# FocoosAI/focoos

Hardware: NVIDIA H100
Metric: images/sec fai-detr-l bs=32 640x640 inference (higher is better)
Workload: dtype f32 (storage and accumulation; every conv/linear product = 3 f16 wgmma products, error ~2^-21)

## Files before the change

focoos_b200/csrc/conv_tc.cu:

```cuda
#include <cuda.h>

#include <cstdlib>
#include <type_traits>

#include "common.cuh"
#include "tma.cuh"
#include "wgmma.cuh"

namespace fb200 {

namespace tc {

constexpr int BLOCK_M = 128;
constexpr int STAGING_BYTES = BLOCK_M * 128;
constexpr int NUM_THREADS = 384;
constexpr int CONSUMER_WARPS = 8;

struct PairOut { __half hi, lo; };
template <typename T> struct is_pair { static constexpr bool value = false; };
template <> struct is_pair<PairOut> { static constexpr bool value = true; };

struct KParams {
  const float* scale; const float* bias; const void* res;
  int act, Cout;
  int KH, KW, pad, cchunks;
  int w_batched;
  int lo_off;
  int w_seg;
  int BW, BH, tiles_w, tiles_h;
  int Ho, Wo;
  int x_pitch;
  int stride2;
  int num_k_blocks;
  int n_tiles, total_tiles;
  float* rowmax;
};

__device__ __forceinline__ void consumer_bar() { asm volatile("bar.sync 1, 256;" ::: "memory"); }

template <int BLOCK_K>
__device__ __forceinline__ uint64_t make_smem_desc(uint32_t smem_addr) {
  uint64_t d = 0;
  d |= (uint64_t)((smem_addr & 0x3FFFFu) >> 4);
  d |= (uint64_t)1 << 16;
  d |= (uint64_t)((8 * BLOCK_K * 2) >> 4) << 32;
  d |= (uint64_t)(BLOCK_K == 64 ? 1 : 2) << 62;
  return d;
}

template <bool GELU>
__device__ __forceinline__ float act1(float v, int act) {
  if constexpr (GELU) return 0.5f * v * (1.f + erff(v * 0.70710678118654752440f));
  switch (act & 15) {
    case FB200_ACT_RELU: return fmaxf(v, 0.f);
    case FB200_ACT_SILU: return __fdividef(v, 1.f + __expf(-v));
    default: return v;
  }
}

__device__ __forceinline__ void atomic_max_float(float* addr, float v) {
  if (v >= 0.f) atomicMax(reinterpret_cast<int*>(addr), __float_as_int(v));
  else atomicMin(reinterpret_cast<unsigned int*>(addr), __float_as_uint(v));
}

struct AccThread {
  int ct;
  int g;
  int r0;
  int cq;
};
__device__ __forceinline__ AccThread acc_thread() {
  const int ct = threadIdx.x - 128, lane = threadIdx.x & 31;
  return {ct, ct >> 7, (ct >> 7) * 64 + ((ct & 127) >> 5) * 16 + (lane >> 2), 2 * (lane & 3)};
}

template <typename TOut>
__device__ __forceinline__ int staging_offset(int row, int lc) {
  if constexpr (is_pair<TOut>::value) return row * 64 + ((((lc >> 3) ^ ((row >> 1) & 3)) << 4) | ((lc & 7) * 2));
  else if constexpr (sizeof(TOut) == 2) return row * 128 + ((((lc >> 3) ^ (row & 7)) << 4) | ((lc & 7) * 2));
  else return row * 128 + ((((lc >> 2) ^ (row & 7)) << 4) | ((lc & 3) * 4));
}

template <typename TOut>
__device__ __forceinline__ void staging_store(uint8_t* stg, int off, float v0, float v1) {
  if constexpr (is_pair<TOut>::value) {
    const __half2 hi = __floats2half2_rn(v0, v1);
    const float2 hf = __half22float2(hi);
    *reinterpret_cast<__half2*>(stg + off) = hi;
    *reinterpret_cast<__half2*>(stg + STAGING_BYTES / 2 + off) = __floats2half2_rn(v0 - hf.x, v1 - hf.y);
  } else if constexpr (sizeof(TOut) == 2) {
    *reinterpret_cast<__half2*>(stg + off) = __floats2half2_rn(v0, v1);
  } else {
    *reinterpret_cast<float2*>(stg + off) = make_float2(v0, v1);
  }
}

template <int NSTG, typename F>
__device__ __forceinline__ void staging_open(int ct, F&& then) {
  if (ct == 0) {
    tma_store_wait_read<NSTG - 1>();
    then();
  }
  consumer_bar();
}
template <typename TOut>
__device__ __forceinline__ void staging_close(int ct, const uint8_t* stg, const CUtensorMap* tmap_d, const CUtensorMap* tmap_d2, int n, int w0, int h0, int img) {
  fence_proxy_async();
  consumer_bar();
  if (ct == 0) {
    tma_store_4d(tmap_d, stg, n, w0, h0, img);
    if constexpr (is_pair<TOut>::value) tma_store_4d(tmap_d2, stg + STAGING_BYTES / 2, n, w0, h0, img);
    tma_store_commit();
  }
}

template <int BLOCK_K, bool FS> __host__ __device__ constexpr int a_stage_bytes() { return (FS ? 2 : 1) * BLOCK_M * BLOCK_K * 2; }
template <int BLOCK_N, int BLOCK_K, bool FS> __host__ __device__ constexpr int b_stage_bytes() { return (FS ? 2 : 1) * BLOCK_N * BLOCK_K * 2; }
template <int BLOCK_N, int STAGES, int BLOCK_K, int NSTG, bool FS> constexpr int smem_bytes() {
  return STAGES * (a_stage_bytes<BLOCK_K, FS>() + b_stage_bytes<BLOCK_N, BLOCK_K, FS>()) + NSTG * STAGING_BYTES + (2 * STAGES + 1) * 8 + 1024 ;
}

template <int BLOCK_N, int STAGES, typename TOut, int BLOCK_K, int NSTG, bool GELU, bool FS>
__global__ void __launch_bounds__(NUM_THREADS, 1)
conv_tc_kernel(const __grid_constant__ CUtensorMap tmap_a, const __grid_constant__ CUtensorMap tmap_b,
               const __grid_constant__ CUtensorMap tmap_d, const __grid_constant__ CUtensorMap tmap_r,
               const __grid_constant__ CUtensorMap tmap_d2, const __grid_constant__ CUtensorMap tmap_r2, const KParams p) {
  constexpr bool PAIR = is_pair<TOut>::value;
  static_assert(BLOCK_K == 32 || BLOCK_K == 64, "one swizzle row per channel chunk");
  extern __shared__ __align__(1024) uint8_t smem_raw[];
  uint8_t* smem = reinterpret_cast<uint8_t*>((reinterpret_cast<uintptr_t>(smem_raw) + 1023) & ~uintptr_t(1023));
  constexpr int A_STAGE_BYTES = a_stage_bytes<BLOCK_K, FS>();
  constexpr int B_STAGE_BYTES = b_stage_bytes<BLOCK_N, BLOCK_K, FS>();
  constexpr int A_HALF = BLOCK_M * BLOCK_K * 2;
  constexpr int B_HALF = BLOCK_N * BLOCK_K * 2;
  uint8_t* smem_a = smem;
  uint8_t* smem_b = smem + STAGES * A_STAGE_BYTES;
  uint8_t* staging = smem_b + STAGES * B_STAGE_BYTES;
  uint64_t* full_bar = reinterpret_cast<uint64_t*>(staging + NSTG * STAGING_BYTES);
  uint64_t* empty_bar = full_bar + STAGES;
  uint64_t* res_bar = empty_bar + STAGES;

  constexpr int CHUNK_COLS = 128 / (int)sizeof(TOut);
  constexpr int NCHUNKS = (BLOCK_N + CHUNK_COLS - 1) / CHUNK_COLS;
  constexpr int RES_SLOTS_A = A_STAGE_BYTES / STAGING_BYTES;
  constexpr int RES_SLOTS = RES_SLOTS_A + B_STAGE_BYTES / STAGING_BYTES;
  constexpr bool RES_RING = RES_SLOTS > 0;
  const bool res_ring = RES_RING && p.res != nullptr && p.rowmax == nullptr;
  auto res_slot = [&](int s, int slot) -> uint8_t* {
    return slot < RES_SLOTS_A ? smem_a + s * A_STAGE_BYTES + slot * STAGING_BYTES : smem_b + s * B_STAGE_BYTES + (slot - RES_SLOTS_A) * STAGING_BYTES;
  };
  auto chunks_of = [&](int n0) { return min(NCHUNKS, (p.Cout - n0 + CHUNK_COLS - 1) / CHUNK_COLS); };

  const int warp = threadIdx.x >> 5, lane = threadIdx.x & 31;
  if (threadIdx.x == 0) {
    asm volatile("prefetch.tensormap [%0];" ::"l"(&tmap_a) : "memory");
    asm volatile("prefetch.tensormap [%0];" ::"l"(&tmap_b) : "memory");
    asm volatile("prefetch.tensormap [%0];" ::"l"(&tmap_d) : "memory");
    for (int i = 0; i < STAGES; ++i) { mbar_init(&full_bar[i], 1); mbar_init(&empty_bar[i], CONSUMER_WARPS); }
    if constexpr (!RES_RING) mbar_init(res_bar, 1);
    fence_barrier_init();
  }
  __syncthreads();
  const int tiles_per_img = p.tiles_w * p.tiles_h;
  struct TileXY { int n0, img, h0, w0; };
  auto tile_of = [&](int t) {
    TileXY r;
    r.n0 = (t % p.n_tiles) * BLOCK_N;
    const int mt = t / p.n_tiles;
    r.img = mt / tiles_per_img;
    const int rem = mt - r.img * tiles_per_img;
    r.h0 = (rem / p.tiles_w) * p.BH;
    r.w0 = (rem % p.tiles_w) * p.BW;
    return r;
  };

  if (warp < 4) {
    if (threadIdx.x != 0) return;
    const uint32_t a_bytes = (uint32_t)(p.BW * p.BH * BLOCK_K * 2);
    auto load_a = [&](uint64_t* bar, void* dst, int c, int kh, int kw, int h0, int w0, int img) {
      if (!p.stride2) {
        tma_load_4d(&tmap_a, bar, dst, c, w0 + kw - p.pad, h0 + kh - p.pad, img);
      } else if (p.stride2 == 2) {
        tma_load_4d(&tmap_a, bar, dst, c, 2 * w0 + kw - p.pad, 2 * h0 + kh - p.pad, img);
      } else {
        const int th = kh - p.pad, tw = kw - p.pad;
        tma_load_5d(&tmap_a, bar, dst, (tw & 1) * p.x_pitch + c, w0 + (tw >> 1), th & 1, h0 + (th >> 1), img);
      }
    };
    auto load_b = [&](uint64_t* bar, void* dst, int k, int n0, int img) {
      if (p.w_batched) tma_load_3d(&tmap_b, bar, dst, k, n0, img);
      else tma_load_2d(&tmap_b, bar, dst, k, n0);
    };
    int stage = 0;
    uint32_t phase = 0;
    for (int t = blockIdx.x; t < p.total_tiles; t += gridDim.x) {
      const TileXY tc = tile_of(t);
      for (int kb = 0; kb < p.num_k_blocks; ++kb) {
        mbar_wait(&empty_bar[stage], phase ^ 1);
        const int tap = kb / p.cchunks, cc = kb - tap * p.cchunks;
        const int kh = tap / p.KW, kw = tap - kh * p.KW;
        uint8_t* dst_a = smem_a + stage * A_STAGE_BYTES;
        uint8_t* dst_b = smem_b + stage * B_STAGE_BYTES;
        if constexpr (FS) {
          const int k_hi = tap * 3 * p.w_seg + cc * BLOCK_K, k_lo = k_hi + p.w_seg;
          mbar_arrive_expect_tx(&full_bar[stage], 2u * a_bytes + (uint32_t)B_STAGE_BYTES);
          load_a(&full_bar[stage], dst_a, cc * BLOCK_K, kh, kw, tc.h0, tc.w0, tc.img);
          load_a(&full_bar[stage], dst_a + A_HALF, p.lo_off + cc * BLOCK_K, kh, kw, tc.h0, tc.w0, tc.img);
          load_b(&full_bar[stage], dst_b, k_hi, tc.n0, tc.img);
          load_b(&full_bar[stage], dst_b + B_HALF, k_lo, tc.n0, tc.img);
        } else {
          mbar_arrive_expect_tx(&full_bar[stage], a_bytes + (uint32_t)B_STAGE_BYTES);
          load_a(&full_bar[stage], dst_a, cc * BLOCK_K, kh, kw, tc.h0, tc.w0, tc.img);
          load_b(&full_bar[stage], dst_b, kb * BLOCK_K, tc.n0, tc.img);
        }
        if (++stage == STAGES) { stage = 0; phase ^= 1; }
      }
      if constexpr (RES_RING) if (res_ring) {
        const int nch = chunks_of(tc.n0);
        for (int ch = 0; ch < nch; ++ch) {
          const int slot = ch % RES_SLOTS;
          if (slot == 0) {
            mbar_wait(&empty_bar[stage], phase ^ 1);
            mbar_arrive_expect_tx(&full_bar[stage], (uint32_t)(min(RES_SLOTS, nch - ch) * p.BW * p.BH * 128));
          }
          uint8_t* dst = res_slot(stage, slot);
          tma_load_4d(&tmap_r, &full_bar[stage], dst, tc.n0 + ch * CHUNK_COLS, tc.w0, tc.h0, tc.img);
          if constexpr (PAIR) tma_load_4d(&tmap_r2, &full_bar[stage], dst + STAGING_BYTES / 2, tc.n0 + ch * CHUNK_COLS, tc.w0, tc.h0, tc.img);
          if (slot == RES_SLOTS - 1 || ch == nch - 1) {
            if (++stage == STAGES) { stage = 0; phase ^= 1; }
          }
        }
      }
    }
    return;
  }

  const AccThread th = acc_thread();
  constexpr int NACC = BLOCK_N / 2;
  const bool post = (p.act & FB200_ACT_RESIDUAL_AFTER) != 0;
  const bool has_res = p.res != nullptr;
  float acc[NACC];
  int stage = 0;
  uint32_t phase = 0, res_phase = 0, chunk_ctr = 0;
  for (int t = blockIdx.x; t < p.total_tiles; t += gridDim.x) {
    const TileXY tc = tile_of(t);
    int prev = -1;
    for (int kb = 0; kb < p.num_k_blocks; ++kb) {
      mbar_wait(&full_bar[stage], phase);
      const uint32_t sa = smem_u32(smem_a + stage * A_STAGE_BYTES) + (uint32_t)(th.g * 64 * BLOCK_K * 2);
      const uint32_t sb = smem_u32(smem_b + stage * B_STAGE_BYTES);
      const uint64_t da = make_smem_desc<BLOCK_K>(sa), db = make_smem_desc<BLOCK_K>(sb);
      wgmma_fence();
#pragma unroll
      for (int k = 0; k < BLOCK_K / 16; ++k) {
        const uint64_t ko = (uint64_t)(k * 2);
        Wgmma<BLOCK_N, 0>::mma(acc, da + ko, db + ko, (kb > 0 || k > 0) ? 1u : 0u);
        if constexpr (FS) {
          const uint64_t da_lo = make_smem_desc<BLOCK_K>(sa + A_HALF), db_lo = make_smem_desc<BLOCK_K>(sb + B_HALF);
          Wgmma<BLOCK_N, 0>::mma(acc, da + ko, db_lo + ko, 1u);
          Wgmma<BLOCK_N, 0>::mma(acc, da_lo + ko, db + ko, 1u);
        }
      }
      wgmma_commit();
      wgmma_wait<1>();
      if (prev >= 0 && lane == 0) mbar_arrive(&empty_bar[prev]);
      prev = stage;
      if (++stage == STAGES) { stage = 0; phase ^= 1; }
    }
    wgmma_wait<0>();
    if (prev >= 0 && lane == 0) mbar_arrive(&empty_bar[prev]);

    auto scale_of = [&](int n) { return (p.scale && n < p.Cout) ? __ldg(p.scale + n) : 1.f; };
    auto bias_of = [&](int n) { return (p.bias && n < p.Cout) ? __ldg(p.bias + n) : 0.f; };
    auto row_valid = [&](int row, int64_t& pix) {
      const int bh = row / p.BW, bw = row - bh * p.BW;
      const int ho = tc.h0 + bh, wo = tc.w0 + bw;
      pix = ((int64_t)tc.img * p.Ho + ho) * p.Wo + wo;
      return row < p.BW * p.BH && ho < p.Ho && wo < p.Wo;
    };
    if (p.rowmax) {
      float m[2] = {-INFINITY, -INFINITY};
#pragma unroll
      for (int j = 0; j < BLOCK_N / 8; ++j) {
#pragma unroll
        for (int e = 0; e < 2; ++e) {
          const int n = tc.n0 + 8 * j + th.cq + e;
          if (n < p.Cout) {
            const float s = scale_of(n), b = bias_of(n);
            m[0] = fmaxf(m[0], fmaf(acc[4 * j + e], s, b));
            m[1] = fmaxf(m[1], fmaf(acc[4 * j + 2 + e], s, b));
          }
        }
      }
#pragma unroll
      for (int h = 0; h < 2; ++h) {
        m[h] = fmaxf(m[h], __shfl_xor_sync(0xffffffffu, m[h], 1));
        m[h] = fmaxf(m[h], __shfl_xor_sync(0xffffffffu, m[h], 2));
        int64_t pix;
        if ((lane & 3) == 0 && row_valid(th.r0 + 8 * h, pix)) atomic_max_float(p.rowmax + pix, m[h]);
      }
      continue;
    }
    const int nch = chunks_of(tc.n0);
#pragma unroll
    for (int ch = 0; ch < NCHUNKS; ++ch) {
      const int c0 = ch * CHUNK_COLS;
      if (ch >= nch) break;
      uint8_t* stg = staging + (chunk_ctr % NSTG) * STAGING_BYTES;
      const uint8_t* res = stg;
      staging_open<NSTG>(th.ct, [&] {
        if constexpr (!RES_RING) if (has_res) {
          mbar_arrive_expect_tx(res_bar, (uint32_t)(p.BW * p.BH * 128));
          tma_load_4d(&tmap_r, res_bar, stg, tc.n0 + c0, tc.w0, tc.h0, tc.img);
          if constexpr (PAIR) tma_load_4d(&tmap_r2, res_bar, stg + STAGING_BYTES / 2, tc.n0 + c0, tc.w0, tc.h0, tc.img);
        }
      });
      if constexpr (RES_RING) {
        if (res_ring) {
          if (ch % RES_SLOTS == 0) mbar_wait(&full_bar[stage], phase);
          res = res_slot(stage, ch % RES_SLOTS);
        }
      } else if (has_res) {
        mbar_wait(res_bar, res_phase);
        res_phase ^= 1;
      }
#pragma unroll
      for (int jj = 0; jj < CHUNK_COLS / 8; ++jj) {
        const int j = c0 / 8 + jj;
        if (j >= BLOCK_N / 8) break;
        const int lc = 8 * jj + th.cq;
        const int n = tc.n0 + c0 + lc;
        const float s0 = scale_of(n), s1 = scale_of(n + 1), b0 = bias_of(n), b1 = bias_of(n + 1);
#pragma unroll
        for (int h = 0; h < 2; ++h) {
          const int row = th.r0 + 8 * h;
          float v0 = fmaf(acc[4 * j + 2 * h], s0, b0), v1 = fmaf(acc[4 * j + 2 * h + 1], s1, b1);
          const int off = staging_offset<TOut>(row, lc);
          auto add_residual = [&]() {
            if (!has_res) return;
            if constexpr (PAIR) {
              const float2 fh = __half22float2(*reinterpret_cast<const __half2*>(res + off));
              const float2 fl = __half22float2(*reinterpret_cast<const __half2*>(res + STAGING_BYTES / 2 + off));
              v0 += fh.x + fl.x;
              v1 += fh.y + fl.y;
            } else if constexpr (sizeof(TOut) == 2) {
              const float2 f = __half22float2(*reinterpret_cast<const __half2*>(res + off));
              v0 += f.x;
              v1 += f.y;
            } else {
              const float2 f = *reinterpret_cast<const float2*>(res + off);
              v0 += f.x;
              v1 += f.y;
            }
          };
          if (!post) add_residual();
          v0 = act1<GELU>(v0, p.act);
          v1 = act1<GELU>(v1, p.act);
          if (post) add_residual();
          staging_store<TOut>(stg, off, v0, v1);
        }
      }
      if constexpr (RES_RING) {
        if (res_ring && (ch % RES_SLOTS == RES_SLOTS - 1 || ch == nch - 1)) {
          __syncwarp();
          if (lane == 0) mbar_arrive(&empty_bar[stage]);
          if (++stage == STAGES) { stage = 0; phase ^= 1; }
        }
      }
      staging_close<TOut>(th.ct, stg, &tmap_d, &tmap_d2, tc.n0 + c0, tc.w0, tc.h0, tc.img);
      ++chunk_ctr;
    }
  }
  if (th.ct == 0) tma_store_wait_all();
}

constexpr int SC_BW = 16, SC_BH = 8;
constexpr int SC_BOX_ROWS = SC_BW * (SC_BH + 2);
constexpr int SC_BOX_BYTES = SC_BOX_ROWS * 64;
constexpr int SC_STAGE_BYTES = 2 * 3 * SC_BOX_BYTES;
constexpr int SC_STAGES = 2;
template <int BLOCK_N> __host__ __device__ constexpr int sc_w_bytes() { return 9 * 2 * BLOCK_N * 64; }
template <int BLOCK_N> constexpr int sc_smem_bytes() {
  return sc_w_bytes<BLOCK_N>() + SC_STAGES * SC_STAGE_BYTES + 2 * STAGING_BYTES + (2 * SC_STAGES + 1) * 8 + 1024 ;
}

template <int BLOCK_N, typename TOut>
__global__ void __launch_bounds__(NUM_THREADS, 1)
conv_tc_smallc_kernel(const __grid_constant__ CUtensorMap tmap_a, const __grid_constant__ CUtensorMap tmap_b,
                      const __grid_constant__ CUtensorMap tmap_d, const __grid_constant__ CUtensorMap tmap_d2, const KParams p) {
  constexpr int W_BYTES = sc_w_bytes<BLOCK_N>();
  constexpr int W_TAP = 2 * BLOCK_N * 64;
  extern __shared__ __align__(1024) uint8_t smem_raw[];
  uint8_t* smem = reinterpret_cast<uint8_t*>((reinterpret_cast<uintptr_t>(smem_raw) + 1023) & ~uintptr_t(1023));
  uint8_t* smem_w = smem;
  uint8_t* smem_a = smem_w + W_BYTES;
  uint8_t* staging = smem_a + SC_STAGES * SC_STAGE_BYTES;
  uint64_t* full_bar = reinterpret_cast<uint64_t*>(staging + 2 * STAGING_BYTES);
  uint64_t* empty_bar = full_bar + SC_STAGES;
  uint64_t* w_bar = empty_bar + SC_STAGES;
  constexpr int CHUNK_COLS = 32;
  constexpr int NCHUNKS = BLOCK_N / CHUNK_COLS;

  const int warp = threadIdx.x >> 5, lane = threadIdx.x & 31;
  if (threadIdx.x == 0) {
    asm volatile("prefetch.tensormap [%0];" ::"l"(&tmap_a) : "memory");
    asm volatile("prefetch.tensormap [%0];" ::"l"(&tmap_d) : "memory");
    for (int i = 0; i < SC_STAGES; ++i) { mbar_init(&full_bar[i], 1); mbar_init(&empty_bar[i], CONSUMER_WARPS); }
    mbar_init(w_bar, 1);
    fence_barrier_init();
  }
  __syncthreads();
  const int tiles_per_img = p.tiles_w * p.tiles_h;
  struct TileXY { int img, h0, w0; };
  auto tile_of = [&](int t) {
    TileXY r;
    r.img = t / tiles_per_img;
    const int rem = t - r.img * tiles_per_img;
    r.h0 = (rem / p.tiles_w) * SC_BH;
    r.w0 = (rem % p.tiles_w) * SC_BW;
    return r;
  };

  if (warp < 4) {
    if (threadIdx.x != 0) return;
    mbar_arrive_expect_tx(w_bar, (uint32_t)W_BYTES);
    for (int tap = 0; tap < 9; ++tap) {
      tma_load_2d(&tmap_b, w_bar, smem_w + tap * W_TAP, tap * 3 * p.w_seg, 0);
      tma_load_2d(&tmap_b, w_bar, smem_w + tap * W_TAP + W_TAP / 2, tap * 3 * p.w_seg + p.w_seg, 0);
    }
    int stage = 0;
    uint32_t phase = 0;
    for (int t = blockIdx.x; t < p.total_tiles; t += gridDim.x) {
      const TileXY tc = tile_of(t);
      mbar_wait(&empty_bar[stage], phase ^ 1);
      mbar_arrive_expect_tx(&full_bar[stage], (uint32_t)SC_STAGE_BYTES);
      uint8_t* dst = smem_a + stage * SC_STAGE_BYTES;
      for (int kw = 0; kw < 3; ++kw) {
        tma_load_4d(&tmap_a, &full_bar[stage], dst + kw * SC_BOX_BYTES, 0, tc.w0 + kw - 1, tc.h0 - 1, tc.img);
        tma_load_4d(&tmap_a, &full_bar[stage], dst + (3 + kw) * SC_BOX_BYTES, p.lo_off, tc.w0 + kw - 1, tc.h0 - 1, tc.img);
      }
      if (++stage == SC_STAGES) { stage = 0; phase ^= 1; }
    }
    return;
  }

  const AccThread th = acc_thread();
  float acc[BLOCK_N / 2];
  float sc[BLOCK_N / 4], bi[BLOCK_N / 4];
#pragma unroll
  for (int j = 0; j < BLOCK_N / 8; ++j)
#pragma unroll
    for (int e = 0; e < 2; ++e) {
      const int n = 8 * j + th.cq + e;
      sc[2 * j + e] = p.scale ? __ldg(p.scale + n) : 1.f;
      bi[2 * j + e] = p.bias ? __ldg(p.bias + n) : 0.f;
    }
  mbar_wait(w_bar, 0);
  const uint32_t sw = smem_u32(smem_w);
  int stage = 0;
  uint32_t phase = 0, chunk_ctr = 0;
  for (int t = blockIdx.x; t < p.total_tiles; t += gridDim.x) {
    const TileXY tc = tile_of(t);
    mbar_wait(&full_bar[stage], phase);
    const uint32_t sa = smem_u32(smem_a + stage * SC_STAGE_BYTES) + (uint32_t)(th.g * 64 * 64);
    wgmma_fence();
#pragma unroll
    for (int tap = 0; tap < 9; ++tap) {
      const int kh = tap / 3, kw = tap - 3 * (tap / 3);
      const uint32_t a_tap = sa + (uint32_t)(kw * SC_BOX_BYTES + kh * SC_BW * 64);
      const uint64_t da = make_smem_desc<32>(a_tap), da_lo = make_smem_desc<32>(a_tap + 3 * SC_BOX_BYTES);
      const uint64_t db = make_smem_desc<32>(sw + tap * W_TAP), db_lo = make_smem_desc<32>(sw + tap * W_TAP + W_TAP / 2);
#pragma unroll
      for (int k = 0; k < 2; ++k) {
        const uint64_t ko = (uint64_t)(k * 2);
        Wgmma<BLOCK_N, 0>::mma(acc, da + ko, db + ko, (tap > 0 || k > 0) ? 1u : 0u);
        Wgmma<BLOCK_N, 0>::mma(acc, da + ko, db_lo + ko, 1u);
        Wgmma<BLOCK_N, 0>::mma(acc, da_lo + ko, db + ko, 1u);
      }
    }
    wgmma_commit();
    wgmma_wait<0>();
    if (lane == 0) mbar_arrive(&empty_bar[stage]);
    if (++stage == SC_STAGES) { stage = 0; phase ^= 1; }

#pragma unroll
    for (int ch = 0; ch < NCHUNKS; ++ch) {
      uint8_t* stg = staging + (chunk_ctr & 1) * STAGING_BYTES;
      staging_open<2>(th.ct, [] {});
#pragma unroll
      for (int jj = 0; jj < CHUNK_COLS / 8; ++jj) {
        const int j = ch * (CHUNK_COLS / 8) + jj;
        const int lc = 8 * jj + th.cq;
#pragma unroll
        for (int h = 0; h < 2; ++h) {
          const int row = th.r0 + 8 * h;
          const float v0 = act1<false>(fmaf(acc[4 * j + 2 * h], sc[2 * j], bi[2 * j]), p.act);
          const float v1 = act1<false>(fmaf(acc[4 * j + 2 * h + 1], sc[2 * j + 1], bi[2 * j + 1]), p.act);
          staging_store<TOut>(stg, staging_offset<TOut>(row, lc), v0, v1);
        }
      }
      staging_close<TOut>(th.ct, stg, &tmap_d, &tmap_d2, ch * CHUNK_COLS, tc.w0, tc.h0, tc.img);
      ++chunk_ctr;
    }
  }
  if (th.ct == 0) tma_store_wait_all();
}

static void choose_tile(int Ho, int Wo, int* BW, int* BH) {
  double best = -1.0;
  for (int bw = 1; bw <= (Wo < 128 ? Wo : 128); ++bw) {
    int bh = 128 / bw;
    if (bh > Ho) bh = Ho;
    if (bh < 1) continue;
    const double tiles = (double)((Wo + bw - 1) / bw) * (double)((Ho + bh - 1) / bh);
    const double eff = (double)Wo * Ho / (tiles * 128.0);
    if (eff > best + 1e-9 || (eff > best - 1e-9 && bw > *BW)) { best = eff; *BW = bw; *BH = bh; }
  }
}

struct OutMaps { CUtensorMap d, d2, r, r2; };
static int encode_out_maps(OutMaps* m, const ConvParams& p, int Wo, int Ho, int B, int BW, int BH, uint64_t batch_stride) {
  const bool pair = p.out_dtype == FB200_F16PAIR, f32 = p.out_dtype == FB200_F32;
  const CUtensorMapDataType dt = f32 ? CU_TENSOR_MAP_DATA_TYPE_FLOAT32 : CU_TENSOR_MAP_DATA_TYPE_FLOAT16;
  const int elt = f32 ? 4 : 2;
  const CUtensorMapSwizzle swz = pair ? CU_TENSOR_MAP_SWIZZLE_64B : CU_TENSOR_MAP_SWIZZLE_128B;
  const uint64_t OP = (uint64_t)p.out_pitch, RP = (uint64_t)p.res_pitch;
  const uint64_t dims[4] = {(uint64_t)p.Cout, (uint64_t)Wo, (uint64_t)Ho, (uint64_t)B};
  const uint64_t str[4] = {1, OP, OP * Wo, batch_stride}, rstr[4] = {1, RP, RP * Wo, RP * Wo * Ho};
  const uint32_t box[4] = {(uint32_t)(pair || f32 ? 32 : 64), (uint32_t)BW, (uint32_t)BH, 1};
  int rc = encode(&m->d, dt, elt, 4, p.out, dims, str, box, pair ? "conv_tc: D(hi)" : "conv_tc: D", swz);
  if (rc) return rc;
  m->d2 = m->d;
  if (pair) rc = encode(&m->d2, dt, elt, 4, static_cast<__half*>(p.out) + p.out_lo_off, dims, str, box, "conv_tc: D(lo)", swz);
  if (rc) return rc;
  m->r = m->d; m->r2 = m->d2;
  if (!p.res) return FB200_OK;
  rc = encode(&m->r, dt, elt, 4, const_cast<void*>(p.res), dims, rstr, box, pair ? "conv_tc: R(hi)" : "conv_tc: R", swz);
  if (rc || !pair) return rc;
  return encode(&m->r2, dt, elt, 4, const_cast<__half*>(static_cast<const __half*>(p.res)) + p.res_lo_off, dims, rstr, box, "conv_tc: R(lo)", swz);
}

static bool smallc_fits(const ConvParams& p) {
  return p.split3 && p.Cin == 3 * 32 && (p.Cout == 32 || p.Cout == 64) && p.KH == 3 && p.KW == 3 && p.stride == 1 && p.pad == 1 &&
         !p.res && !p.rowmax && p.w_bs == 0 && (p.out_dtype == FB200_F32 || p.out_dtype == FB200_F16PAIR);
}

static int conv2d_tc_smallc(const ConvParams& p, cudaStream_t st) {
  KParams kp{};
  kp.scale = p.scale; kp.bias = p.bias; kp.act = p.act; kp.Cout = p.Cout;
  kp.lo_off = (int)p.x_lo_off;
  kp.w_seg = 32;
  kp.tiles_w = (p.Wo + SC_BW - 1) / SC_BW; kp.tiles_h = (p.Ho + SC_BH - 1) / SC_BH; kp.Ho = p.Ho; kp.Wo = p.Wo;
  const int64_t total = (int64_t)p.B * kp.tiles_w * kp.tiles_h;
  if (total > 0x7fffffffLL) { set_error("conv_tc: too many tiles (%lld)", (long long)total); return FB200_ERR_UNSUPPORTED; }
  kp.total_tiles = (int)total;
  CUtensorMap ta, tb;
  OutMaps om;
  const uint64_t P = (uint64_t)p.x_pitch;
  {
    const uint64_t dims[4] = {(uint64_t)kp.lo_off + 32, (uint64_t)p.W, (uint64_t)p.H, (uint64_t)p.B};
    const uint64_t str[4] = {1, P, P * p.W, P * p.W * p.H};
    const uint32_t box[4] = {32, SC_BW, SC_BH + 2, 1};
    int rc = encode(&ta, CU_TENSOR_MAP_DATA_TYPE_FLOAT16, 2, 4, const_cast<void*>(p.x), dims, str, box, "conv_tc: A(patch)", CU_TENSOR_MAP_SWIZZLE_64B);
    if (rc) return rc;
  }
  {
    const uint64_t dims[2] = {(uint64_t)p.K, (uint64_t)p.Cout};
    const uint64_t str[2] = {1, (uint64_t)p.K};
    const uint32_t box[2] = {32, (uint32_t)p.Cout};
    int rc = encode(&tb, CU_TENSOR_MAP_DATA_TYPE_FLOAT16, 2, 2, const_cast<void*>(p.w), dims, str, box, "conv_tc: W", CU_TENSOR_MAP_SWIZZLE_64B);
    if (rc) return rc;
  }
  if (int rc = encode_out_maps(&om, p, p.Wo, p.Ho, p.B, SC_BW, SC_BH, (uint64_t)p.out_bs)) return rc;
  auto run = [&](auto blockn_tag, auto out_tag) -> int {
    constexpr int BN_ = decltype(blockn_tag)::value;
    return launch_persistent<conv_tc_smallc_kernel<BN_, decltype(out_tag)>, sc_smem_bytes<BN_>()>("conv_tc_smallc_kernel", kp.total_tiles, NUM_THREADS, st, ta, tb,
                                                                                                 om.d, om.d2, kp);
  };
  typedef std::integral_constant<int, 32> N32;
  typedef std::integral_constant<int, 64> N64;
  const bool outp = p.out_dtype == FB200_F16PAIR;
  if (p.Cout == 32) return outp ? run(N32{}, PairOut{}) : run(N32{}, float{});
  return outp ? run(N64{}, PairOut{}) : run(N64{}, float{});
}

}

bool conv2d_tc_supported(const ConvParams& p, int x_dtype, int out_dtype) {
  if (x_dtype != FB200_F16) return false;
  if (out_dtype != FB200_F16 && out_dtype != FB200_F32 && out_dtype != FB200_F16PAIR) return false;
  if (p.split3 && out_dtype == FB200_F16) return false;
  const int Clog = p.split3 ? p.Cin / 3 : p.Cin;
  if (out_dtype == FB200_F16PAIR) {
    if (!p.split3 || p.rowmax || p.w_bs != 0 || p.Cout % 8 != 0) return false;
    if ((p.out_lo_off * 2) % 16 != 0 || (p.out_pitch * 2) % 16 != 0 || (p.out_bs * 2) % 16 != 0) return false;
    if (p.res && ((p.res_lo_off * 2) % 16 != 0 || (p.res_pitch * 2) % 16 != 0 || p.Cout % 32 != 0)) return false;
  }
  if (p.split3 && (p.x_lo_off * 2) % 16 != 0) return false;
  if (Clog % 32 != 0 || p.x_pitch % 8 != 0) return false;
  if (p.split3 && p.Cin % 3 != 0) return false;
  if ((reinterpret_cast<uintptr_t>(p.x) | reinterpret_cast<uintptr_t>(p.w) | reinterpret_cast<uintptr_t>(p.out)) & 15) return false;
  const int oelt = out_dtype == FB200_F32 ? 4 : 2;
  if ((p.out_pitch * oelt) % 16 != 0) return false;
  if (!p.rowmax && (p.Cout * oelt) % 16 != 0) return false;
  if (p.res && ((p.res_pitch * oelt) % 16 != 0 || (reinterpret_cast<uintptr_t>(p.res) & 15))) return false;
  if (p.res && out_dtype != FB200_F16PAIR && p.Cout % (128 / oelt) != 0) return false;
  if (p.KH != p.KW) return false;
  if (p.w_bs != 0 && (p.w_bs * 2) % 16 != 0) return false;
  if ((p.act & 15) == FB200_ACT_GELU && (out_dtype != FB200_F16 || Clog % 64 != 0)) return false;
  if ((p.act & 15) == FB200_ACT_SIGMOID) return false;
  if ((p.out_bs * oelt) % 16 != 0) return false;
  if (p.stride == 1) return (2 * p.pad == p.KH - 1) || (p.KH == 1 && p.pad == 0);
  if (p.stride == 2) {
    if (p.KH == 3 && p.pad == 1) return true;
    return p.KH == 2 && p.pad == 0 && p.H % 2 == 0 && p.W % 2 == 0;
  }
  return false;
}

int conv2d_tc(const ConvParams& p, cudaStream_t st) {
  using namespace tc;
  if (smallc_fits(p)) return conv2d_tc_smallc(p, st);
  KParams kp;
  kp.scale = p.scale; kp.bias = p.bias; kp.res = p.res; kp.act = p.act; kp.Cout = p.Cout;
  kp.KH = p.KH; kp.KW = p.KW; kp.pad = p.pad;
  const int Clog = p.split3 ? p.Cin / 3 : p.Cin;
  const int BK = (Clog % 64 == 0) ? 64 : 32;
  kp.lo_off = p.split3 ? (int)p.x_lo_off : Clog;
  kp.w_seg = Clog;
  const CUtensorMapSwizzle swz = BK == 64 ? CU_TENSOR_MAP_SWIZZLE_128B : CU_TENSOR_MAP_SWIZZLE_64B;
  kp.cchunks = Clog / BK; kp.x_pitch = p.x_pitch;
  kp.stride2 = (p.stride != 2) ? 0 : (p.H % 2 == 0 && p.W % 2 == 0) ? 1 : 2;
  kp.num_k_blocks = p.KH * p.KW * kp.cchunks;
  int B = p.B, H = p.H, W = p.W, Ho = p.Ho, Wo = p.Wo;
  const bool flat = (p.KH == 1 && p.stride == 1 && p.out_bs == (int64_t)p.Ho * p.Wo * p.out_pitch) && p.w_bs == 0;
  kp.w_batched = p.w_bs != 0 ? 1 : 0;
  kp.rowmax = p.rowmax;
  if (flat) {
    if (p.M > 0x7fffffffLL) { set_error("conv_tc: M too large"); return FB200_ERR_UNSUPPORTED; }
    W = Wo = (int)p.M; H = Ho = 1; B = 1;
  }
  int BW = 1, BH = 1;
  choose_tile(Ho, Wo, &BW, &BH);
  kp.BW = BW; kp.BH = BH; kp.tiles_w = (Wo + BW - 1) / BW; kp.tiles_h = (Ho + BH - 1) / BH; kp.Ho = Ho; kp.Wo = Wo;
  const int64_t m_tiles = (int64_t)B * kp.tiles_w * kp.tiles_h;

  CUtensorMap ta, tb;
  OutMaps om;
  int rc;
  const uint64_t P = (uint64_t)p.x_pitch;
  if (!kp.stride2) {
    const uint64_t dims[4] = {(uint64_t)(p.split3 ? kp.lo_off + Clog : p.Cin), (uint64_t)W, (uint64_t)H, (uint64_t)B};
    const uint64_t str[4] = {1, P, P * W, P * W * H};
    const uint32_t box[4] = {(uint32_t)BK, (uint32_t)BW, (uint32_t)BH, 1};
    rc = encode(&ta, CU_TENSOR_MAP_DATA_TYPE_FLOAT16, 2, 4, const_cast<void*>(p.x), dims, str, box, "conv_tc: A", swz);
  } else if (kp.stride2 == 2) {
    const uint64_t dims[4] = {(uint64_t)(p.split3 ? kp.lo_off + Clog : p.Cin), (uint64_t)W, (uint64_t)H, (uint64_t)B};
    const uint64_t str[4] = {1, P, P * W, P * W * H};
    const uint32_t box[4] = {(uint32_t)BK, 2 * (uint32_t)BW, 2 * (uint32_t)BH, 1};
    const uint32_t estr[4] = {1, 2, 2, 1};
    rc = encode(&ta, CU_TENSOR_MAP_DATA_TYPE_FLOAT16, 2, 4, const_cast<void*>(p.x), dims, str, box, "conv_tc: A(s2 odd)", swz, estr);
  } else {
    const uint64_t dims[5] = {2 * P, (uint64_t)W / 2, 2, (uint64_t)H / 2, (uint64_t)B};
    const uint64_t str[5] = {1, 2 * P, P * W, 2 * P * W, P * W * H};
    const uint32_t box[5] = {(uint32_t)BK, (uint32_t)BW, 1, (uint32_t)BH, 1};
    rc = encode(&ta, CU_TENSOR_MAP_DATA_TYPE_FLOAT16, 2, 5, const_cast<void*>(p.x), dims, str, box, "conv_tc: A(s2)", swz);
  }
  if (rc) return rc;
  rc = encode_out_maps(&om, p, Wo, Ho, B, BW, BH, flat ? (uint64_t)p.out_pitch * Wo * Ho : (uint64_t)p.out_bs);
  if (rc) return rc;

  auto run = [&](auto blockn_tag, auto stages_tag, auto bk_tag, auto gelu_tag, auto fs_tag) -> int {
    constexpr bool FS_ = decltype(fs_tag)::value;
    constexpr int BN_ = decltype(blockn_tag)::value;
    constexpr int ST_ = decltype(stages_tag)::value;
    constexpr int BK_ = decltype(bk_tag)::value;
    constexpr int NS_ = 2;
    {
      const uint64_t dims[3] = {(uint64_t)p.K, (uint64_t)p.Cout, (uint64_t)p.B};
      const uint64_t str[3] = {1, (uint64_t)p.K, (uint64_t)p.w_bs};
      const uint32_t box[3] = {(uint32_t)BK_, (uint32_t)BN_, 1};
      int r2 = encode(&tb, CU_TENSOR_MAP_DATA_TYPE_FLOAT16, 2, p.w_bs ? 3 : 2, const_cast<void*>(p.w), dims, str, box, "conv_tc: W", swz);
      if (r2) return r2;
    }
    kp.n_tiles = (p.Cout + BN_ - 1) / BN_;
    const int64_t total = m_tiles * kp.n_tiles;
    if (total > 0x7fffffffLL) { set_error("conv_tc: too many tiles (%lld)", (long long)total); return FB200_ERR_UNSUPPORTED; }
    kp.total_tiles = (int)total;
    auto launch = [&](auto out_tag) -> int {
      return launch_persistent<conv_tc_kernel<BN_, ST_, decltype(out_tag), BK_, NS_, decltype(gelu_tag)::value, FS_>, smem_bytes<BN_, ST_, BK_, NS_, FS_>()>(
          "conv_tc_kernel", kp.total_tiles, NUM_THREADS, st, ta, tb, om.d, om.r, om.d2, om.r2, kp);
    };
    const bool outp = p.out_dtype == FB200_F16PAIR;
    if constexpr (decltype(gelu_tag)::value) return launch(__half{});
    else if constexpr (FS_) return outp ? launch(PairOut{}) : launch(float{});
    else {
      if (outp) { set_error("conv_tc: pair output is only produced by the fused-split configurations"); return FB200_ERR_UNSUPPORTED; }
      return p.out_dtype == FB200_F16 ? launch(__half{}) : launch(float{});
    }
  };
  using std::integral_constant;
  typedef std::false_type NF;
  typedef std::true_type FS;
  typedef integral_constant<int, 64> K64;
  typedef integral_constant<int, 32> K32;
  typedef integral_constant<int, 128> N128;
  typedef integral_constant<int, 64> N64;
  typedef integral_constant<int, 4> S4;
  typedef integral_constant<int, 3> S3;
  if ((p.act & 15) == FB200_ACT_GELU)
    return run(N128{}, S4{}, K64{}, std::true_type{}, NF{});
  if (p.split3) {
    if (BK == 64) {
      if (p.Cout > 64) return run(N128{}, S3{}, K64{}, std::false_type{}, FS{});
      return run(N64{}, S4{}, K64{}, std::false_type{}, FS{});
    }
    if (p.Cout > 64) return run(N128{}, S4{}, K32{}, std::false_type{}, FS{});
    return run(N64{}, S4{}, K32{}, std::false_type{}, FS{});
  }
  if (BK == 32) {
    if (p.Cout > 64) return run(N128{}, S4{}, K32{}, std::false_type{}, NF{});
    return run(N64{}, S4{}, K32{}, std::false_type{}, NF{});
  }
  if (p.Cout > 64) return run(N128{}, S4{}, K64{}, std::false_type{}, NF{});
  return run(N64{}, S4{}, K64{}, std::false_type{}, NF{});
}

}
```

focoos_b200/csrc/wgmma.cuh:

```cuda
#pragma once
#include <stdint.h>

namespace fb200 {

__device__ __forceinline__ void wgmma_fence() { asm volatile("wgmma.fence.sync.aligned;" ::: "memory"); }
__device__ __forceinline__ void wgmma_commit() { asm volatile("wgmma.commit_group.sync.aligned;" ::: "memory"); }
template <int N> __device__ __forceinline__ void wgmma_wait() { asm volatile("wgmma.wait_group.sync.aligned %0;" ::"n"(N) : "memory"); }

template <int N, int TRANS> struct Wgmma;

template <int TRANS> struct Wgmma<32, TRANS> {
  static __device__ __forceinline__ void mma(float (&d)[16], uint64_t a, uint64_t b, uint32_t scale_d) {
    asm volatile(
        "{\n\t.reg .pred p;\n\t"
        "setp.ne.b32 p, %18, 0;\n\t"
        "wgmma.mma_async.sync.aligned.m64n32k16.f32.f16.f16 "
        "{%0, %1, %2, %3, %4, %5, %6, %7, %8, %9, %10, %11, %12, %13, %14, %15}, "
        "%16, %17, p, 1, 1, %19, %19;\n\t}"
        : "+f"(d[0]), "+f"(d[1]), "+f"(d[2]), "+f"(d[3]), "+f"(d[4]), "+f"(d[5]), "+f"(d[6]), "+f"(d[7]),
          "+f"(d[8]), "+f"(d[9]), "+f"(d[10]), "+f"(d[11]), "+f"(d[12]), "+f"(d[13]), "+f"(d[14]), "+f"(d[15])
        : "l"(a), "l"(b), "r"(scale_d), "n"(TRANS));
  }
};

template <int TRANS> struct Wgmma<64, TRANS> {
  static __device__ __forceinline__ void mma(float (&d)[32], uint64_t a, uint64_t b, uint32_t scale_d) {
    asm volatile(
        "{\n\t.reg .pred p;\n\t"
        "setp.ne.b32 p, %34, 0;\n\t"
        "wgmma.mma_async.sync.aligned.m64n64k16.f32.f16.f16 "
        "{%0, %1, %2, %3, %4, %5, %6, %7, %8, %9, %10, %11, %12, %13, %14, %15, "
        "%16, %17, %18, %19, %20, %21, %22, %23, %24, %25, %26, %27, %28, %29, %30, %31}, "
        "%32, %33, p, 1, 1, %35, %35;\n\t}"
        : "+f"(d[0]), "+f"(d[1]), "+f"(d[2]), "+f"(d[3]), "+f"(d[4]), "+f"(d[5]), "+f"(d[6]), "+f"(d[7]),
          "+f"(d[8]), "+f"(d[9]), "+f"(d[10]), "+f"(d[11]), "+f"(d[12]), "+f"(d[13]), "+f"(d[14]), "+f"(d[15]),
          "+f"(d[16]), "+f"(d[17]), "+f"(d[18]), "+f"(d[19]), "+f"(d[20]), "+f"(d[21]), "+f"(d[22]), "+f"(d[23]),
          "+f"(d[24]), "+f"(d[25]), "+f"(d[26]), "+f"(d[27]), "+f"(d[28]), "+f"(d[29]), "+f"(d[30]), "+f"(d[31])
        : "l"(a), "l"(b), "r"(scale_d), "n"(TRANS));
  }
};

template <int TRANS> struct Wgmma<128, TRANS> {
  static __device__ __forceinline__ void mma(float (&d)[64], uint64_t a, uint64_t b, uint32_t scale_d) {
    asm volatile(
        "{\n\t.reg .pred p;\n\t"
        "setp.ne.b32 p, %66, 0;\n\t"
        "wgmma.mma_async.sync.aligned.m64n128k16.f32.f16.f16 "
        "{%0, %1, %2, %3, %4, %5, %6, %7, %8, %9, %10, %11, %12, %13, %14, %15, "
        "%16, %17, %18, %19, %20, %21, %22, %23, %24, %25, %26, %27, %28, %29, %30, %31, "
        "%32, %33, %34, %35, %36, %37, %38, %39, %40, %41, %42, %43, %44, %45, %46, %47, "
        "%48, %49, %50, %51, %52, %53, %54, %55, %56, %57, %58, %59, %60, %61, %62, %63}, "
        "%64, %65, p, 1, 1, %67, %67;\n\t}"
        : "+f"(d[0]), "+f"(d[1]), "+f"(d[2]), "+f"(d[3]), "+f"(d[4]), "+f"(d[5]), "+f"(d[6]), "+f"(d[7]),
          "+f"(d[8]), "+f"(d[9]), "+f"(d[10]), "+f"(d[11]), "+f"(d[12]), "+f"(d[13]), "+f"(d[14]), "+f"(d[15]),
          "+f"(d[16]), "+f"(d[17]), "+f"(d[18]), "+f"(d[19]), "+f"(d[20]), "+f"(d[21]), "+f"(d[22]), "+f"(d[23]),
          "+f"(d[24]), "+f"(d[25]), "+f"(d[26]), "+f"(d[27]), "+f"(d[28]), "+f"(d[29]), "+f"(d[30]), "+f"(d[31]),
          "+f"(d[32]), "+f"(d[33]), "+f"(d[34]), "+f"(d[35]), "+f"(d[36]), "+f"(d[37]), "+f"(d[38]), "+f"(d[39]),
          "+f"(d[40]), "+f"(d[41]), "+f"(d[42]), "+f"(d[43]), "+f"(d[44]), "+f"(d[45]), "+f"(d[46]), "+f"(d[47]),
          "+f"(d[48]), "+f"(d[49]), "+f"(d[50]), "+f"(d[51]), "+f"(d[52]), "+f"(d[53]), "+f"(d[54]), "+f"(d[55]),
          "+f"(d[56]), "+f"(d[57]), "+f"(d[58]), "+f"(d[59]), "+f"(d[60]), "+f"(d[61]), "+f"(d[62]), "+f"(d[63])
        : "l"(a), "l"(b), "r"(scale_d), "n"(TRANS));
  }
};

}
```

Baseline: 891.1.

## Feed split-precision conv A operand from registers via ldmatrix and RS wgmma

For the three-product split-f16 path with BLOCK_N=128, A hi/lo fragments are now loaded into registers with ldmatrix and the wgmmas use the register-sourced A form, so each A fragment is read from shared memory once and reused across two products. Each k-step is committed and waited separately with double-buffered fragments, and the empty-barrier release moves after the first step. The goal is less shared-memory descriptor traffic for A. The cost is more register pressure, an extra commit/wait per k-step that may serialize wgmma issue, and reliance on the ldmatrix addressing matching the swizzled staging layout.

```diff
diff --git a/focoos_b200/csrc/conv_tc.cu b/focoos_b200/csrc/conv_tc.cu
--- a/focoos_b200/csrc/conv_tc.cu
+++ b/focoos_b200/csrc/conv_tc.cu
@@ -118,6 +118,25 @@
 template <int BLOCK_N, int BLOCK_K, bool FS> __host__ __device__ constexpr int b_stage_bytes() { return (FS ? 2 : 1) * BLOCK_N * BLOCK_K * 2; }
 template <int BLOCK_N, int STAGES, int BLOCK_K, int NSTG, bool FS> constexpr int smem_bytes() {
   return STAGES * (a_stage_bytes<BLOCK_K, FS>() + b_stage_bytes<BLOCK_N, BLOCK_K, FS>()) + NSTG * STAGING_BYTES + (2 * STAGES + 1) * 8 + 1024 ;
+}
+
+template <int BLOCK_K>
+__device__ __forceinline__ uint32_t a_frag_offset(int row0, int k, int lane) {
+  typedef std::conditional_t<BLOCK_K == 64, __half, PairOut> Layout;
+  return (uint32_t)staging_offset<Layout>(row0 + (lane & 15), 16 * k + 8 * (lane >> 4));
+}
+
+template <int BLOCK_N>
+__device__ __forceinline__ void fs_step(float (&acc)[BLOCK_N / 2], uint32_t (&fr)[2][4], uint32_t a_hi, uint32_t a_lo, uint64_t db_hi, uint64_t db_lo,
+                                        uint32_t scale_d) {
+  ldmatrix_x4(fr[0], a_hi);
+  ldmatrix_x4(fr[1], a_lo);
+  wgmma_fence();
+  WgmmaRS<BLOCK_N>::mma(acc, fr[0], db_hi, scale_d);
+  WgmmaRS<BLOCK_N>::mma(acc, fr[0], db_lo, 1u);
+  WgmmaRS<BLOCK_N>::mma(acc, fr[1], db_hi, 1u);
+  wgmma_commit();
+  wgmma_wait<1>();
 }
 
 template <int BLOCK_N, int STAGES, typename TOut, int BLOCK_K, int NSTG, bool GELU, bool FS>
@@ -240,6 +259,8 @@
   const bool post = (p.act & FB200_ACT_RESIDUAL_AFTER) != 0;
   const bool has_res = p.res != nullptr;
   float acc[NACC];
+  constexpr bool RS = FS && BLOCK_N == 128;
+  uint32_t frag[2][2][4];
   int stage = 0;
   uint32_t phase = 0, res_phase = 0, chunk_ctr = 0;
   for (int t = blockIdx.x; t < p.total_tiles; t += gridDim.x) {
@@ -249,21 +270,33 @@
       mbar_wait(&full_bar[stage], phase);
       const uint32_t sa = smem_u32(smem_a + stage * A_STAGE_BYTES) + (uint32_t)(th.g * 64 * BLOCK_K * 2);
       const uint32_t sb = smem_u32(smem_b + stage * B_STAGE_BYTES);
-      const uint64_t da = make_smem_desc<BLOCK_K>(sa), db = make_smem_desc<BLOCK_K>(sb);
-      wgmma_fence();
-#pragma unroll
-      for (int k = 0; k < BLOCK_K / 16; ++k) {
-        const uint64_t ko = (uint64_t)(k * 2);
-        Wgmma<BLOCK_N, 0>::mma(acc, da + ko, db + ko, (kb > 0 || k > 0) ? 1u : 0u);
-        if constexpr (FS) {
-          const uint64_t da_lo = make_smem_desc<BLOCK_K>(sa + A_HALF), db_lo = make_smem_desc<BLOCK_K>(sb + B_HALF);
-          Wgmma<BLOCK_N, 0>::mma(acc, da + ko, db_lo + ko, 1u);
-          Wgmma<BLOCK_N, 0>::mma(acc, da_lo + ko, db + ko, 1u);
-        }
-      }
-      wgmma_commit();
-      wgmma_wait<1>();
-      if (prev >= 0 && lane == 0) mbar_arrive(&empty_bar[prev]);
+      const uint64_t db = make_smem_desc<BLOCK_K>(sb);
+      if constexpr (RS) {
+        const uint64_t db_lo = make_smem_desc<BLOCK_K>(sb + B_HALF);
+        const int row0 = ((th.ct & 127) >> 5) * 16;
+#pragma unroll
+        for (int k = 0; k < BLOCK_K / 16; ++k) {
+          const uint32_t ao = a_frag_offset<BLOCK_K>(row0, k, lane);
+          fs_step<BLOCK_N>(acc, frag[k & 1], sa + ao, sa + A_HALF + ao, db + (uint64_t)(k * 2), db_lo + (uint64_t)(k * 2), (kb > 0 || k > 0) ? 1u : 0u);
+          if (k == 0 && prev >= 0 && lane == 0) mbar_arrive(&empty_bar[prev]);
+        }
+      } else {
+        const uint64_t da = make_smem_desc<BLOCK_K>(sa);
+        wgmma_fence();
+#pragma unroll
+        for (int k = 0; k < BLOCK_K / 16; ++k) {
+          const uint64_t ko = (uint64_t)(k * 2);
+          Wgmma<BLOCK_N, 0>::mma(acc, da + ko, db + ko, (kb > 0 || k > 0) ? 1u : 0u);
+          if constexpr (FS) {
+            const uint64_t da_lo = make_smem_desc<BLOCK_K>(sa + A_HALF), db_lo = make_smem_desc<BLOCK_K>(sb + B_HALF);
+            Wgmma<BLOCK_N, 0>::mma(acc, da + ko, db_lo + ko, 1u);
+            Wgmma<BLOCK_N, 0>::mma(acc, da_lo + ko, db + ko, 1u);
+          }
+        }
+        wgmma_commit();
+        wgmma_wait<1>();
+        if (prev >= 0 && lane == 0) mbar_arrive(&empty_bar[prev]);
+      }
       prev = stage;
       if (++stage == STAGES) { stage = 0; phase ^= 1; }
     }
diff --git a/focoos_b200/csrc/wgmma.cuh b/focoos_b200/csrc/wgmma.cuh
--- a/focoos_b200/csrc/wgmma.cuh
+++ b/focoos_b200/csrc/wgmma.cuh
@@ -63,4 +63,64 @@
   }
 };
 
+template <int N> struct WgmmaRS;
+
+template <> struct WgmmaRS<32> {
+  static __device__ __forceinline__ void mma(float (&d)[16], const uint32_t (&a)[4], uint64_t b, uint32_t scale_d) {
+    asm volatile(
+        "{\n\t.reg .pred p;\n\t"
+        "setp.ne.b32 p, %21, 0;\n\t"
+        "wgmma.mma_async.sync.aligned.m64n32k16.f32.f16.f16 "
+        "{%0, %1, %2, %3, %4, %5, %6, %7, %8, %9, %10, %11, %12, %13, %14, %15}, "
+        "{%16, %17, %18, %19}, %20, p, 1, 1, 0;\n\t}"
+        : "+f"(d[0]), "+f"(d[1]), "+f"(d[2]), "+f"(d[3]), "+f"(d[4]), "+f"(d[5]), "+f"(d[6]), "+f"(d[7]),
+          "+f"(d[8]), "+f"(d[9]), "+f"(d[10]), "+f"(d[11]), "+f"(d[12]), "+f"(d[13]), "+f"(d[14]), "+f"(d[15])
+        : "r"(a[0]), "r"(a[1]), "r"(a[2]), "r"(a[3]), "l"(b), "r"(scale_d));
+  }
+};
+
+template <> struct WgmmaRS<64> {
+  static __device__ __forceinline__ void mma(float (&d)[32], const uint32_t (&a)[4], uint64_t b, uint32_t scale_d) {
+    asm volatile(
+        "{\n\t.reg .pred p;\n\t"
+        "setp.ne.b32 p, %37, 0;\n\t"
+        "wgmma.mma_async.sync.aligned.m64n64k16.f32.f16.f16 "
+        "{%0, %1, %2, %3, %4, %5, %6, %7, %8, %9, %10, %11, %12, %13, %14, %15, "
+        "%16, %17, %18, %19, %20, %21, %22, %23, %24, %25, %26, %27, %28, %29, %30, %31}, "
+        "{%32, %33, %34, %35}, %36, p, 1, 1, 0;\n\t}"
+        : "+f"(d[0]), "+f"(d[1]), "+f"(d[2]), "+f"(d[3]), "+f"(d[4]), "+f"(d[5]), "+f"(d[6]), "+f"(d[7]),
+          "+f"(d[8]), "+f"(d[9]), "+f"(d[10]), "+f"(d[11]), "+f"(d[12]), "+f"(d[13]), "+f"(d[14]), "+f"(d[15]),
+          "+f"(d[16]), "+f"(d[17]), "+f"(d[18]), "+f"(d[19]), "+f"(d[20]), "+f"(d[21]), "+f"(d[22]), "+f"(d[23]),
+          "+f"(d[24]), "+f"(d[25]), "+f"(d[26]), "+f"(d[27]), "+f"(d[28]), "+f"(d[29]), "+f"(d[30]), "+f"(d[31])
+        : "r"(a[0]), "r"(a[1]), "r"(a[2]), "r"(a[3]), "l"(b), "r"(scale_d));
+  }
+};
+
+template <> struct WgmmaRS<128> {
+  static __device__ __forceinline__ void mma(float (&d)[64], const uint32_t (&a)[4], uint64_t b, uint32_t scale_d) {
+    asm volatile(
+        "{\n\t.reg .pred p;\n\t"
+        "setp.ne.b32 p, %69, 0;\n\t"
+        "wgmma.mma_async.sync.aligned.m64n128k16.f32.f16.f16 "
+        "{%0, %1, %2, %3, %4, %5, %6, %7, %8, %9, %10, %11, %12, %13, %14, %15, "
+        "%16, %17, %18, %19, %20, %21, %22, %23, %24, %25, %26, %27, %28, %29, %30, %31, "
+        "%32, %33, %34, %35, %36, %37, %38, %39, %40, %41, %42, %43, %44, %45, %46, %47, "
+        "%48, %49, %50, %51, %52, %53, %54, %55, %56, %57, %58, %59, %60, %61, %62, %63}, "
+        "{%64, %65, %66, %67}, %68, p, 1, 1, 0;\n\t}"
+        : "+f"(d[0]), "+f"(d[1]), "+f"(d[2]), "+f"(d[3]), "+f"(d[4]), "+f"(d[5]), "+f"(d[6]), "+f"(d[7]),
+          "+f"(d[8]), "+f"(d[9]), "+f"(d[10]), "+f"(d[11]), "+f"(d[12]), "+f"(d[13]), "+f"(d[14]), "+f"(d[15]),
+          "+f"(d[16]), "+f"(d[17]), "+f"(d[18]), "+f"(d[19]), "+f"(d[20]), "+f"(d[21]), "+f"(d[22]), "+f"(d[23]),
+          "+f"(d[24]), "+f"(d[25]), "+f"(d[26]), "+f"(d[27]), "+f"(d[28]), "+f"(d[29]), "+f"(d[30]), "+f"(d[31]),
+          "+f"(d[32]), "+f"(d[33]), "+f"(d[34]), "+f"(d[35]), "+f"(d[36]), "+f"(d[37]), "+f"(d[38]), "+f"(d[39]),
+          "+f"(d[40]), "+f"(d[41]), "+f"(d[42]), "+f"(d[43]), "+f"(d[44]), "+f"(d[45]), "+f"(d[46]), "+f"(d[47]),
+          "+f"(d[48]), "+f"(d[49]), "+f"(d[50]), "+f"(d[51]), "+f"(d[52]), "+f"(d[53]), "+f"(d[54]), "+f"(d[55]),
+          "+f"(d[56]), "+f"(d[57]), "+f"(d[58]), "+f"(d[59]), "+f"(d[60]), "+f"(d[61]), "+f"(d[62]), "+f"(d[63])
+        : "r"(a[0]), "r"(a[1]), "r"(a[2]), "r"(a[3]), "l"(b), "r"(scale_d));
+  }
+};
+
+__device__ __forceinline__ void ldmatrix_x4(uint32_t (&r)[4], uint32_t addr) {
+  asm volatile("ldmatrix.sync.aligned.m8n8.x4.shared.b16 {%0, %1, %2, %3}, [%4];" : "=r"(r[0]), "=r"(r[1]), "=r"(r[2]), "=r"(r[3]) : "r"(addr) : "memory");
 }
+
+}
```

New measurement: 917.9, median of 6. 1.03x the previous value.
